# OnurBasci/Real_Time_Path_Tracing_With_SpatioTemporal_Filtering

Measured on AMD Instinct MI355X. Metric: Mray/s (closest-hit queries / whole-frame time: G-buffer + gradient + trace + a-trous), higher is better.
Workload: dtype f32

## Files before the change

### real_time_path_tracing_with_spatiotemporal_filtering_amd/csrc/api_context.hip

```cpp
#include "api_internal.hpp"

#include <atomic>

namespace rtpt_impl {

thread_local std::string g_err;

int fail(int code, const std::string& msg) {
  g_err = msg;
  return code;
}


size_t frame_blocks(const rtpt_ctx* c) {
  const size_t tiles = ((static_cast<size_t>(c->cfg.width) + 63) / 64) * ((static_cast<size_t>(c->cfg.row_end - c->cfg.row_begin) + 3) / 4);
  return std::max(tiles, static_cast<size_t>(c->n_cu > 0 ? c->n_cu : 256) * 8);
}
int ensure_stack_spill(rtpt_ctx* c, size_t blocks) {
  if (!c->scene.use_bvh) return RTPT_OK;
  const size_t depth = static_cast<size_t>(c->scene.tree.bvh_depth + 2 < 8 ? 8 : c->scene.tree.bvh_depth + 2);
  const size_t lds = std::min<size_t>(depth, static_cast<size_t>(c->bvh_stack_lds));
  if (depth <= lds || blocks <= c->stack_spill_blocks) return RTPT_OK;
  if (c->stack_spill.ptr) {
    hipError_t e = hipStreamSynchronize(c->stream);
// ... 111 lines not shown
  g.row_base = static_cast<int32_t>(c->cfg.row_begin);
  g.y0 = static_cast<int32_t>(y0);
  g.y1 = static_cast<int32_t>(y1);
  return g;
}

rt::SceneView scene_view(const rtpt_ctx* c) {
  rt::SceneView s;
  s.isect_id = static_cast<const float4*>(c->scene.isect_id.ptr);
  s.isect_leaf = static_cast<const float4*>(c->scene.isect_leaf.ptr);
  s.leaf_ids = static_cast<const uint32_t*>(c->scene.tree.leaf_order.ptr);
  s.shade = static_cast<const float4*>(c->scene.shade.ptr);
  s.nodes = static_cast<const rt::BvhNodeQ*>(c->scene.tree.nodes.ptr);
  s.bvh_grid = static_cast<const float*>(c->scene.bvh_grid_dev.ptr);
  s.n_tris = c->scene.n_tris;
  s.use_bvh = c->scene.use_bvh ? 1u : 0u;
  s.paired = (c->scene.tris_paired && !c->no_pairing) ? 1u : 0u;
  s.leaf_pairs = c->scene.tree.leaf_pairs ? 1u : 0u;
  s.stack_depth = static_cast<uint32_t>(c->scene.tree.bvh_depth + 2 < 8 ? 8 : c->scene.tree.bvh_depth + 2);
  s.stack_lds = std::min<uint32_t>(s.stack_depth, static_cast<uint32_t>(c->bvh_stack_lds));
  s.stack_spill = static_cast<uint32_t*>(c->stack_spill.ptr);
  s.materials = static_cast<const float4*>(c->scene.materials.ptr);
  s.n_base_tris = c->scene.n_base_tris ? c->scene.n_base_tris : 1u;
  return s;
}

rt::TexView tex_view(const rtpt_ctx* c) {
  rt::TexView t;
  t.records = static_cast<const float4*>(c->scene.textures.records.ptr);
  t.desc = static_cast<const rt::TexDesc*>(c->scene.textures.desc.ptr);
  t.texels = static_cast<const float4*>(c->scene.textures.texels.ptr);
  t.levels = static_cast<const uint32_t*>(c->scene.textures.levels.ptr);
  t.bounce_spread = c->tex_bounce_spread;
  return t;
}

bool screen_bounds(const rtpt_ctx* c, const double org[3], const double c0[3], const double c1[3], const double c2[3],
                   double p00, double p11, double jitter_px, rt::TriBounds* out) {
  if (c->scene.host_tris.empty() || c->scene.n_tris > static_cast<uint32_t>(rt::kCullMaxTris)) return false;
  const double W = c->cfg.width, H = c->cfg.height;
  for (uint32_t t = 0; t < c->scene.n_tris; t++) {
    double xmin = 1e30, xmax = -1e30, ymin = 1e30, ymax = -1e30;
    bool unbounded = false;
    for (int k = 0; k < 3; k++) {
      const float* P = c->scene.host_tris.data() + 9 * static_cast<size_t>(t) + 3 * k;
      const double r[3] = {P[0] - org[0], P[1] - org[1], P[2] - org[2]};
// ... 139 lines not shown
    HIP_TRY(hipSetDevice(dev));
  }
  rtpt_ctx* c = new (std::nothrow) rtpt_ctx();
  if (!c) return fail(RTPT_E_NOMEM, "host allocation failed");
  c->cfg = *cfg;
  c->device = dev;
  hipError_t e = hipStreamCreateWithFlags(&c->own_stream, hipStreamNonBlocking);
  if (e != hipSuccess) {
    delete c;
    return fail(RTPT_E_DEVICE, std::string("hipStreamCreate: ") + hipGetErrorString(e));
  }
  c->stream = c->own_stream;
  {
    hipDeviceProp_t prop;
    if (hipGetDeviceProperties(&prop, dev) == hipSuccess && prop.multiProcessorCount > 0) c->n_cu = prop.multiProcessorCount;
    e = rt::prepare_device_atrous();
    if (e == hipSuccess) e = rt::prepare_device_atrous_chain();
    if (e != hipSuccess) {
      rtpt_destroy(c);
      return fail(RTPT_E_DEVICE, std::string("hipFuncSetAttribute: ") + hipGetErrorString(e));
    }
  }
  if (const char* v = std::getenv("RTPT_NO_TRI_PAIRS")) c->no_pairing = std::atoi(v) != 0;
  if (const char* v = std::getenv("RTPT_HOST_REFIT")) c->host_refit = std::atoi(v) != 0;
  c->device_bvh = (cfg->flags & RTPT_FLAG_DEVICE_BVH_BUILD) != 0;
  c->device_bvh_sah = c->device_bvh && (cfg->flags & RTPT_FLAG_DEVICE_BVH_SAH) != 0;
  if (const char* v = std::getenv("RTPT_DEVICE_BVH")) {
    if (!std::strcmp(v, "sah"))
      c->device_bvh = c->device_bvh_sah = true;
    else
      c->device_bvh = c->device_bvh || std::atoi(v) != 0;
  }
  c->device_flatten = c->device_bvh && (cfg->flags & RTPT_FLAG_DEVICE_FLATTEN) != 0;
  if (const char* v = std::getenv("RTPT_LBVH_ORDER")) c->lbvh_by_height = !std::strcmp(v, "height");
  if (const char* v = std::getenv("RTPT_NO_TRACE_FUSION")) c->fuse_trace = std::atoi(v) == 0;
  if (const char* v = std::getenv("RTPT_NO_FRAME_REUSE")) c->frame_reuse = std::atoi(v) == 0;
  if (const char* v = std::getenv("RTPT_NO_REPROJ_REUSE")) c->reproj_reuse = std::atoi(v) == 0;
  if (const char* v = std::getenv("RTPT_TRACE_POOL")) c->trace_pool = std::atoi(v) != 0;
  if (const char* v = std::getenv("RTPT_TEX_BOUNCE_SPREAD")) {
    const float f = std::strtof(v, nullptr);
    if (f > 0.0f && f <= 64.0f) c->tex_bounce_spread = f;
  }
  if (const char* v = std::getenv("RTPT_PT_WINDOW")) c->trace_window = static_cast<uint32_t>(std::max(0, std::atoi(v)));
  if (const char* v = std::getenv("RTPT_CHAIN_G1")) c->filter_policy.chain_g_pin = std::atoi(v);
  if (const char* v = std::getenv("RTPT_CHAIN_GENERIC")) c->filter_policy.chain_generic = std::atoi(v);
  if (const char* v = std::getenv("RTPT_CHAIN_WG_PER_CU")) c->filter_policy.chain_wg_per_cu = std::atoi(v);
// ... 337 lines not shown
```

### real_time_path_tracing_with_spatiotemporal_filtering_amd/csrc/api_internal.hpp

```cpp
#pragma once
#include <hip/hip_runtime.h>

#include <algorithm>
#include <cmath>
#include <cstdio>
#include <cstdlib>
#include <cfloat>
#include <cstring>
#include <new>
#include <string>
#include <vector>

#include "../../include/rtpt.h"
#include "bvh.hpp"
#include "kernels.hpp"
#include "rtpt_math.hpp"


namespace rtpt_impl {


extern thread_local std::string g_err;
int fail(int code, const std::string& msg);

// ... 159 lines not shown
  int device = 0;
  int n_cu = 256;
  hipStream_t own_stream = nullptr;
  hipStream_t stream = nullptr;

  Buf color[4];
  Buf vis[2];
  int lut_cur = 0;
  Buf worldpos, gradient, depth, prev_pixel, hit_id, raycount;
  Buf moments[2], variance[2];
  Buf var_scale;
  Buf albedo, shaded;
  Buf path_queue[2], path_queue_count;
  Buf normals;
  FrameState frame;
  void* present_dst = nullptr;
  Rows present_rows;
  Buf ray_tab;
  float ray_tab_p00 = 0.f, ray_tab_p11 = 0.f;
  uint32_t ray_tab_w = 0, ray_tab_h = 0;

  Scene scene;
  bool no_pairing = false;
  bool host_refit = false;
  bool device_bvh = false;
  bool device_bvh_sah = false;
  bool lbvh_by_height = false;
  bool device_flatten = false;
  Buf bvh_build_scratch, bvh_build_header;
  hipEvent_t build_ev[2] = {nullptr, nullptr};
  Buf pair_word;
  struct XfStage {
    void* host = nullptr;
    size_t bytes = 0;
    hipEvent_t done = nullptr;
    bool pending = false;
  } xf_stage[2];
  int xf_stage_cur = 0;
  uint64_t upload_info[4] = {0, 0, 0, 0};

  bool tables_valid = false;
  uint32_t debug_mask = 0;
  hipEvent_t handoff_event = nullptr;

  rt::GbufferArgs pending_gb{};
  bool pending_gb_valid = false;
// ... 108 lines not shown
```

### real_time_path_tracing_with_spatiotemporal_filtering_amd/csrc/bvh.cpp

```cpp
#include "bvh.hpp"

#include <algorithm>
#include <cfloat>
#include <cmath>
#include <cstring>

namespace rt {
namespace {

struct Box {
  float mn[3], mx[3];
  void reset() {
    for (int a = 0; a < 3; a++) {
      mn[a] = FLT_MAX;
      mx[a] = -FLT_MAX;
    }
  }
  void grow(const float* p) {
    for (int a = 0; a < 3; a++) {
      mn[a] = std::min(mn[a], p[a]);
      mx[a] = std::max(mx[a], p[a]);
    }
  }
  void grow(const Box& b) {
// ... 3 lines not shown
    }
  }
  float half_area() const {
    float dx = mx[0] - mn[0], dy = mx[1] - mn[1], dz = mx[2] - mn[2];
    if (dx < 0.f) return 0.f;
    return dx * dy + dy * dz + dz * dx;
  }
};

struct Prim {
  Box box;
  float c[3];
  uint32_t id;
  uint32_t w;
};

struct Child {
  Box box;
  uint32_t idx;
  uint32_t cnt;
};

constexpr int kBins = kBvhBins;

struct Builder {
  std::vector<Prim> prims;
  Bvh* out;
  float pad;

  Child make_leaf(uint32_t lo, uint32_t hi) {
    Child c;
    c.box.reset();
    c.idx = static_cast<uint32_t>(out->leaf_order.size());
    c.cnt = 0;
    for (uint32_t i = lo; i < hi; i++) {
      c.box.grow(prims[i].box);
      for (uint32_t k = 0; k < prims[i].w; k++) out->leaf_order.push_back(prims[i].id + k);
      c.cnt += prims[i].w;
    }
    return c;
  }

  Child build(uint32_t lo, uint32_t hi, int depth) {
    out->max_depth = std::max(out->max_depth, depth);
    const uint32_t w = prims[lo].w;
    uint32_t n = (hi - lo) * w;
// ... 4 lines not shown
    cb.reset();
    bb.reset();
    for (uint32_t i = lo; i < hi; i++) {
      cb.grow(prims[i].c);
      bb.grow(prims[i].box);
    }
    uint32_t mid = lo;
    bool median = depth >= kBvhMaxDepth - 26;
    if (median && may_leaf) return make_leaf(lo, hi);
    if (!median) {
      float best_cost = FLT_MAX;
      int best_axis = -1, best_split = -1;
      for (int a = 0; a < 3; a++) {
        float ext = cb.mx[a] - cb.mn[a];
        if (!(ext > 0.f)) continue;
        Box bins[kBins];
        uint32_t cnt[kBins];
        for (int b = 0; b < kBins; b++) {
          bins[b].reset();
          cnt[b] = 0;
        }
        float scale = kBins / ext;
        for (uint32_t i = lo; i < hi; i++) {
          int b = std::min(kBins - 1, static_cast<int>((prims[i].c[a] - cb.mn[a]) * scale));
          bins[b].grow(prims[i].box);
          cnt[b] += w;
        }
        float right_area[kBins];
        uint32_t right_cnt[kBins];
        Box acc;
        acc.reset();
        uint32_t c = 0;
        for (int b = kBins - 1; b > 0; b--) {
          acc.grow(bins[b]);
          c += cnt[b];
          right_area[b] = acc.half_area();
          right_cnt[b] = c;
        }
        acc.reset();
        c = 0;
        for (int b = 0; b < kBins - 1; b++) {
          acc.grow(bins[b]);
          c += cnt[b];
          if (c == 0 || right_cnt[b + 1] == 0) continue;
          float cost = acc.half_area() * c + right_area[b + 1] * right_cnt[b + 1];
          if (cost < best_cost) {
            best_cost = cost;
            best_axis = a;
            best_split = b;
          }
        }
      }
      if (may_leaf && (best_axis < 0 || kNodeCost * bb.half_area() + best_cost >= static_cast<float>(n) * bb.half_area()))
        return make_leaf(lo, hi);
      if (best_axis >= 0) {
        float ext = cb.mx[best_axis] - cb.mn[best_axis];
        float scale = kBins / ext;
        float mn = cb.mn[best_axis];
        int axis = best_axis, split = best_split;
        auto it = std::partition(prims.begin() + lo, prims.begin() + hi, [&](const Prim& p) {
          int b = std::min(kBins - 1, static_cast<int>((p.c[axis] - mn) * scale));
          return b <= split;
        });
        mid = static_cast<uint32_t>(it - prims.begin());
      }
    }
    if (mid == lo || mid == hi) {
      int axis = 0;
      float best = -1.f;
      for (int a = 0; a < 3; a++) {
        float e = cb.mx[a] - cb.mn[a];
        if (e > best) {
          best = e;
          axis = a;
        }
      }
      mid = lo + (hi - lo) / 2;
      std::nth_element(prims.begin() + lo, prims.begin() + mid, prims.begin() + hi,
                       [axis](const Prim& x, const Prim& y) {
                         return x.c[axis] < y.c[axis] || (x.c[axis] == y.c[axis] && x.id < y.id);
                       });
    }

    uint32_t node_index = static_cast<uint32_t>(out->nodes.size());
// ... 192 lines not shown
```

### real_time_path_tracing_with_spatiotemporal_filtering_amd/csrc/closest_hit.hpp

```cpp
#pragma once

#include "device_common.hpp"

namespace rt {
namespace {

struct HitRec {
  float t;
  uint32_t id1;
  float u, v, ad;
};

#define RTPT_DIV_TH(a, b) ((a) / (b))
#define RTPT_DIV_SH(a, b) ((a) / (b))

#ifndef RTPT_TRACE_ITEMS
#define RTPT_TRACE_ITEMS 11
#endif

template <bool TIE_BREAK>
__device__ __forceinline__ void tri_test(f3 o, f3 d, float4 r0, float4 r1, float4 r2, uint32_t id1, HitRec& h) {
  f3 v0{r0.x, r0.y, r0.z}, e1{r0.w, r1.x, r1.y}, e2{r1.z, r1.w, r2.x}, n{r2.y, r2.z, r2.w};
  f3 tv = o - v0;
  const float dn = exact::dot(d, n);
// ... 90 lines not shown
  }
  {
    const float dn = exact::dot(d, nb);
    const uint32_t sm = f2u(dn) & 0x80000000u;
    const float tt = u2f(f2u(exact::dot(tv, nb)) ^ sm);
    const float u = u2f(f2u(exact::dot(e2b, c)) ^ sm);
    const float v = u2f(f2u(e2c) ^ sm);
    const float ad = __builtin_fabsf(dn);
    if ((u <= 0.0f) && (v >= 0.0f) && (v - u <= ad) && (tt < 0.0f)) {
      const float th = RTPT_DIV_TH(-tt, ad);
      bool better = th < h.t;
      better = better || (th == h.t && h.id1 != 0 && id1b < h.id1);
      if (better) {
        h.t = th;
        h.id1 = id1b;
        h.u = u;
        h.v = v;
        h.ad = ad;
      }
    }
  }
}

__device__ __forceinline__ void closest_hit_brute(const SceneView& sc, f3 o, f3 d, HitRec& h) {
  typedef float v4f __attribute__((ext_vector_type(4)));
  using cv4f = const __attribute__((address_space(4))) v4f;
  cv4f* rec = (cv4f*)sc.isect_id;
  const uint32_t n = sc.n_tris;
  constexpr int kBruteUnroll = 8;
  constexpr int kPairUnroll = 8;
  if (sc.paired) {
#pragma unroll kPairUnroll
    for (uint32_t i = 0; i < n; i += 2) {
      const v4f a0 = rec[3 * i], a1 = rec[3 * i + 1], a2 = rec[3 * i + 2], b1 = rec[3 * i + 4], b2 = rec[3 * i + 5];
      tri_pair_test(o, d, make_float4(a0.x, a0.y, a0.z, a0.w), make_float4(a1.x, a1.y, a1.z, a1.w), make_float4(a2.x, a2.y, a2.z, a2.w),
                    make_float4(b1.x, b1.y, b1.z, b1.w), make_float4(b2.x, b2.y, b2.z, b2.w), i + 1, h);
    }
    return;
  }
#pragma unroll kBruteUnroll
  for (uint32_t i = 0; i < n; i++) {
    const v4f a0 = rec[3 * i], a1 = rec[3 * i + 1], a2 = rec[3 * i + 2];
    tri_test<false>(o, d, make_float4(a0.x, a0.y, a0.z, a0.w), make_float4(a1.x, a1.y, a1.z, a1.w),
                    make_float4(a2.x, a2.y, a2.z, a2.w), i + 1, h);
  }
}

constexpr int kWaveW = 16, kWaveH = 4;
__device__ __forceinline__ uint32_t tile_pixel(int wave, uint32_t lane) {
  return ((lane >> 4) << 6) | (static_cast<uint32_t>(wave) << 4) | (lane & 15u);
}
__device__ __forceinline__ int wave_x0(int wave) { return kWaveW * wave; }
__device__ __forceinline__ unsigned long long span_candidates(const TriBounds* bounds, uint32_t n, int x0, int y0) {
// ... 150 lines not shown
      cur = cl;
    } else if (hr) {
      cur = cr;
    } else {
      cur = pop();
    }
  };
  while (cur != kSentinel) {
    while (true) {
      const bool walk = !(cur & kLeafBit);
      const unsigned long long mw = __ballot(walk);
      if (!mw) break;
      const int nw = __builtin_popcountll(mw), na = __builtin_popcountll(__ballot(true));
      if (na - nw >= kBvhLeafRatio * nw) break;
      if (walk) node_step();
    }
    if ((cur & kLeafBit) && cur != kSentinel) {
      test_leaf(cur);
      cur = pop();
    }
  }
}

template <int BVH>
__device__ __forceinline__ void closest_hit(const SceneView& sc, f3 o, f3 d, HitRec& h, uint32_t* stack, int tid,
                                            int nt = kThreads, int bucket = 0) {
  if (BVH)
    closest_hit_bvh<BVH == 2>(sc, o, d, h, stack, tid, nt, bucket);
  else
    closest_hit_brute(sc, o, d, h);
}

__device__ __forceinline__ f3 bary_point(f3 v0, f3 v1, f3 v2, float b0, float b1, float b2) {
  return f3{fmaf_(v2.x, b2, fmaf_(v1.x, b1, v0.x * b0)), fmaf_(v2.y, b2, fmaf_(v1.y, b1, v0.y * b0)),
            fmaf_(v2.z, b2, fmaf_(v1.z, b1, v0.z * b0))};
}

inline int scene_mode(const SceneView& sc) { return sc.use_bvh ? (sc.leaf_pairs ? 2 : 1) : 0; }

}
}
```

### real_time_path_tracing_with_spatiotemporal_filtering_amd/csrc/kernels.hip

```cpp
#include <cstdlib>

#include "atrous_comb.hpp"
#include "final_split.hpp"
#include "pathtrace_tile.hpp"
#include "select.hpp"

namespace rt {
namespace {

__global__ void k_scene_prepare(ScenePrepArgs a) {
  uint32_t i = blockIdx.x * blockDim.x + threadIdx.x;
  if (i >= a.n_tris) return;
  {
    const float* t = a.tris + 9 * static_cast<size_t>(i);
    f3 v0 = ld3(t), v1 = ld3(t + 3), v2 = ld3(t + 6);
    f3 e1 = v1 - v0, e2 = v2 - v0;
    f3 nn = exact::cross(e1, e2);
    a.isect_id[3 * i] = make_float4(v0.x, v0.y, v0.z, e1.x);
    a.isect_id[3 * i + 1] = make_float4(e1.y, e1.z, e2.x, e2.y);
    a.isect_id[3 * i + 2] = make_float4(e2.z, nn.x, nn.y, nn.z);
    f3 n = exact::normalize(nn);
    a.shade[3 * i] = make_float4(v0.x, v0.y, v0.z, n.x);
    a.shade[3 * i + 1] = make_float4(v1.x, v1.y, v1.z, n.y);
    a.shade[3 * i + 2] = make_float4(v2.x, v2.y, v2.z, n.z);
// ... 69 lines not shown
#if RTPT_TILE_TIMELINE
  TimelineScope tl_(0, blockIdx.y * gridDim.x + blockIdx.x);
#endif
  gbuffer_tile<BVH>(a, blockIdx.x, blockIdx.y, stack);
}

__global__ __launch_bounds__(kThreads) void k_gradient(GradientArgs a) {
  const int x = blockIdx.x * kBlockX + threadIdx.x;
  const int y = a.g.y0 + blockIdx.y * kBlockY + threadIdx.y;
  if (x >= a.g.W || y >= a.g.y1) return;
  const size_t i = static_cast<size_t>(y - a.g.row_base) * a.g.W + x;
  const uint32_t id = a.vis[i];
  const f3 wp = id ? xyz(a.worldpos[i]) : f3{0.f, 0.f, 0.f};
  store_gradient(a.grad, i, gradient_lambda(id, wp, a.lut, a.lut_prev, a.normal_tab, a.area_tab, ld3(a.cam), ld3(a.light), ld3(a.light_prev), ld3(a.color),
                                            ld3(a.color_prev)));
}

template <int BVH, bool COMPACT, bool DEMOD, int TEX, int SPEC>
__global__ __launch_bounds__(kPtThreads)
__attribute__((amdgpu_waves_per_eu(kPtBvhWaves, kPtBvhWaves)))
void k_pathtrace(PathtraceArgs a, TexView tex) {
  pathtrace_tile<BVH, COMPACT, false, DEMOD, TEX, SPEC>(a, tex);
}
template <bool COMPACT, bool DEMOD, int TEX, int SPEC>
__global__ __launch_bounds__(kPtThreads)
__attribute__((amdgpu_waves_per_eu(kPtWaves, kPtWaves)))
void k_pathtrace_small(PathtraceArgs a, TexView tex) {
  pathtrace_tile<0, COMPACT, false, DEMOD, TEX, SPEC>(a, tex);
}

template <int BVH, bool DEMOD, int TEX, int SPEC>
__global__ __launch_bounds__(kPtThreads)
__attribute__((amdgpu_waves_per_eu(kPtBvhWaves, kPtBvhWaves)))
void k_gbuffer_pathtrace(PathtraceArgs a, GbufferArgs g, TexView tex) {
  gbuffer_pathtrace_body<BVH, DEMOD, TEX, SPEC>(a, g, tex);
}
template <bool DEMOD, int TEX, int SPEC>
__global__ __launch_bounds__(kPtThreads)
__attribute__((amdgpu_waves_per_eu(kPtWaves, kPtWaves)))
void k_gbuffer_pathtrace_small(PathtraceArgs a, GbufferArgs g, TexView tex) {
  gbuffer_pathtrace_body<0, DEMOD, TEX, SPEC>(a, g, tex);
}

template <int CW>
__global__ __launch_bounds__(kPtThreads)
__attribute__((amdgpu_waves_per_eu(kPtWaves, kPtWaves)))
void k_pathtrace_final(PathtraceArgs a, TexView tex, AtrousArgs f, FinalSplit sp) {
  static_assert(kPtThreads == kShThreads && kPtRows == kShWaves, "the two bodies share the workgroup shape");
  const FinalRole r = final_role(sp, blockIdx.x);
  if (r.role == kFinalRoleTile) {
    pathtrace_tile<0, true, false, false, 0, 0, 1>(a, tex, r.index, sp.tiles_x, a.tiles_y);
  } else {
    extern __shared__ __attribute__((aligned(16))) unsigned char final_lds[];
    const bool front = r.role == kFinalRoleFront;
#if RTPT_TILE_TIMELINE
    FilterTimelineScope tl_(r.role, front ? r.index : sp.n_front + r.index);
#endif
    comb_items<CW, true, false, false, 1, false, false, true, true>(f, final_lds, r.index, front ? sp.n_front : sp.n_tail,
                                                                       front ? 0u : sp.front_items, front ? sp.front_items : sp.items);
  }
}

template <int BVH, int TEX, int SPEC>
__global__ __launch_bounds__(kPtThreads) void k_pathtrace_queue(PathtraceArgs a, TexView tex) {
  extern __shared__ __attribute__((aligned(16))) uint32_t stack[];
  PathState& st = *reinterpret_cast<PathState*>(stack);
  __shared__ uint32_t wave_cnt[kPtRows];
  __shared__ uint32_t q_base;
  __shared__ unsigned int block_rays;
  const int tid = threadIdx.y * kBlockX + threadIdx.x;
  const int wave = __builtin_amdgcn_readfirstlane(static_cast<int>(threadIdx.y));
  const uint32_t lane = threadIdx.x;
  if (tid == 0) block_rays = 0;
  const f3 light_c = ld3(a.light_c);
  const uint32_t region = blockIdx.x % kPathQueues;
  const uint32_t n_in = a.q_in_count[region];
  const size_t region_base = static_cast<size_t>(region) * a.queue_region;
  unsigned int rays = 0;
  for (uint32_t base = (blockIdx.x / kPathQueues) * kPtThreads; base < n_in; base += (gridDim.x / kPathQueues) * kPtThreads) {
    uint32_t pix = 0, rng = 0;
    f3 o{0.f, 0.f, 0.f}, d{0.f, 0.f, -1.f}, acc{1.f, 1.f, 1.f};
    bool alive = base + static_cast<uint32_t>(tid) < n_in;
    if (alive) {
      const float4* q = reinterpret_cast<const float4*>(a.q_in) + 3 * (region_base + base + tid);
      const float4 q0 = q[0], q1 = q[1], q2 = q[2];
      pix = __float_as_uint(q0.x);
      rng = __float_as_uint(q0.y);
      o = f3{q0.z, q0.w, q1.x};
      d = f3{q1.y, q1.z, q1.w};
      acc = f3{q2.x, q2.y, q2.z};
    }
    for (uint32_t seg = a.seg_begin; seg < a.seg_end; seg++) {
      if (alive) {
        HitRec h{a.tmax, 0u, 0.f, 0.f, 1.f};
        closest_hit<BVH>(a.scene, o, d, h, stack, tid, kPtThreads, 1 + static_cast<int>(seg));
        const int x = static_cast<int>(pix & 0xFFFFu), y = static_cast<int>(pix >> 16);
        if (y >= a.count_y0 && y < a.count_y1) rays++;
        if (shade_segment<TEX, BVH, (RTPT_TRACE_ITEMS & 8) && BVH == 0, SPEC>(a, h, seg, light_c, o, d, acc, rng, tex)) {
          alive = false;
          const size_t gi = static_cast<size_t>(y - a.g.row_base) * a.g.W + x;
          a.image[gi] = make_float4(acc.x, acc.y, acc.z, a.depth[gi]);
        }
      }
      if (seg + 1 >= a.seg_end) break;
      const unsigned long long live = __ballot(alive);
      if (lane == 0) wave_cnt[wave] = static_cast<uint32_t>(__builtin_popcountll(live));
      __syncthreads();
      uint32_t cbase = 0, total = 0;
#pragma unroll
      for (int w = 0; w < kPtRows; w++) {
        const uint32_t c = wave_cnt[w];
        if (w < wave) cbase += c;
        total += c;
      }
      if (total == 0) break;
      if (alive) {
        const uint32_t slot = cbase + __builtin_amdgcn_mbcnt_hi(static_cast<uint32_t>(live >> 32),
                                                              __builtin_amdgcn_mbcnt_lo(static_cast<uint32_t>(live), 0u));
// ... 102 lines not shown
  size_t dyn = stack_bytes > sizeof(PathState) ? stack_bytes : sizeof(PathState);
  if (fin) {
    if (gb || !pol || !fin->reproj_in || !pathtrace_takes_final(a, tex, specular)) std::abort();
    dyn = dyn > final_role_lds(*fin) ? dyn : final_role_lds(*fin);
  }
  PathtraceArgs b = a;
  b.tiles_y = tiles_y;
  b.multi_off = static_cast<uint32_t>(dyn / 4);
  const size_t dyn_queue = dyn;
  if (a.spp > 1) dyn += 4 * kPtThreads * 4;
  const uint32_t phase0 = a.first_window ? a.first_window : pt_first_window(a.scene.use_bvh != 0);
  const bool split = a.spp == 1 && a.compact && a.queue[0] && a.queue_count && a.max_segments > phase0 &&
                     (a.max_segments <= 2 * phase0 || a.queue[1]);
  b.seg_begin = 0;
  b.seg_end = split ? phase0 : a.max_segments;
  b.q_in = nullptr;
  b.q_in_count = nullptr;
  b.q_out = split ? a.queue[0] : nullptr;
  b.q_out_count = split ? a.queue_count : nullptr;
  if (split) (void)hipMemsetAsync(a.queue_count, 0, 2 * kPathQueues * sizeof(uint32_t), s);
  if (fin) {
    const FinalSplit sp = final_split(a, *fin, *pol, grid.x, tiles_y);
    const dim3 grid1(final_grid(sp));
    hipLaunchKernelGGL(k_pathtrace_final<kFinalRoleCw>, grid1, block, dyn, s, b, tex, *fin, sp);
  } else
#if RTPT_AB_VARIANTS
  if (pool) {
    if (gb)
      hipLaunchKernelGGL((k_pathtrace_pool<true>), grid, block, dyn, s, b, *gb);
    else
      hipLaunchKernelGGL((k_pathtrace_pool<false>), grid, block, dyn, s, b, GbufferArgs{});
  } else
#endif
  with_mode3(scene_mode(a.scene), [&](auto mode) {
    constexpr int M = decltype(mode)::value;
    with_bool(a.albedo != nullptr, [&](auto demod) {
      constexpr bool D = decltype(demod)::value;
      with_mode3(tex_mode(tex), [&](auto tmode) {
        constexpr int T = decltype(tmode)::value;
        with_mode3(spec_mode(specular), [&](auto spec) {
          constexpr int S = decltype(spec)::value;
          if (gb) {
            if constexpr (M != 0)
              hipLaunchKernelGGL((k_gbuffer_pathtrace<M, D, T, S>), grid, block, dyn, s, b, *gb, tex);
            else
              hipLaunchKernelGGL((k_gbuffer_pathtrace_small<D, T, S>), grid, block, dyn, s, b, *gb, tex);
            return;
          }
          with_bool(a.compact != 0, [&](auto compact) {
            constexpr bool C = decltype(compact)::value;
            if constexpr (M != 0)
              hipLaunchKernelGGL((k_pathtrace<M, C, D, T, S>), grid, block, dyn, s, b, tex);
            else
              hipLaunchKernelGGL((k_pathtrace_small<C, D, T, S>), grid, block, dyn, s, b, tex);
          });
        });
      });
    });
  });
  if (!split) return;
  const int n_cu = a.n_cu > 0 ? a.n_cu : 256;
  const dim3 qgrid(static_cast<uint32_t>(n_cu) * 8u);
  int cur = 0;
  for (uint32_t begin = phase0, len = phase0; begin < a.max_segments; begin += len, len *= 2, cur ^= 1) {
    const uint32_t end = begin + len < a.max_segments ? begin + len : a.max_segments;
    PathtraceArgs c = b;
    c.seg_begin = begin;
    c.seg_end = end;
    c.q_in = a.queue[cur];
    c.q_in_count = a.queue_count + cur * kPathQueues;
    const bool more = end < a.max_segments;
    c.q_out = more ? a.queue[cur ^ 1] : nullptr;
    c.q_out_count = more ? a.queue_count + (cur ^ 1) * kPathQueues : nullptr;
    if (more) (void)hipMemsetAsync(a.queue_count + (cur ^ 1) * kPathQueues, 0, kPathQueues * sizeof(uint32_t), s);
    with_mode3(scene_mode(a.scene), [&](auto mode) {
      with_mode3(tex_mode(tex), [&](auto tmode) {
        with_mode3(spec_mode(specular), [&](auto spec) {
          hipLaunchKernelGGL((k_pathtrace_queue<decltype(mode)::value, decltype(tmode)::value, decltype(spec)::value>), qgrid, block,
                             dyn_queue, s, c, tex);
        });
      });
    });
    if (end >= a.max_segments) break;
  }
}

}
```

### real_time_path_tracing_with_spatiotemporal_filtering_amd/csrc/kernels.hpp

```cpp
#pragma once

#include <hip/hip_runtime.h>
#include <stdint.h>

#include "bvh.hpp"
#include "texture.hpp"

namespace rt {

struct SceneView {
  const float4* isect_id;
  const float4* isect_leaf;
  const uint32_t* leaf_ids;
  const float4* shade;
  const BvhNodeQ* nodes;
  const float* bvh_grid;
  uint32_t n_tris;
  uint32_t use_bvh;
  uint32_t paired;
  uint32_t leaf_pairs;
  uint32_t stack_depth;
  uint32_t stack_lds;
  uint32_t* stack_spill;
  const float4* materials;
  uint32_t n_base_tris;
};

struct TexView {
  const float4* records;
  const TexDesc* desc;
  const float4* texels;
  const uint32_t* levels;
  float bounce_spread;
};

void launch_mip_downsample(float4* atlas, uint32_t src, uint32_t sw, uint32_t sh, uint32_t dst, hipStream_t s);

struct TriBounds {
  int16_t x0, y0, x1, y1;
};
constexpr int kCullMaxTris = 64;

struct FrameGeom {
  int32_t W, H;
  int32_t row_base;
  int32_t y0, y1;
};

struct GbufferArgs {
// ... 264 lines not shown
```

### real_time_path_tracing_with_spatiotemporal_filtering_amd/csrc/pathtrace_tile.hpp

```cpp
#pragma once

#include "gbuffer_tile.hpp"
#include "shade_segment.hpp"

namespace rt {
namespace {

constexpr int kPtRows = 4;
constexpr int kPtThreads = kBlockX * kPtRows;

__device__ __forceinline__ void enqueue_paths(const PathtraceArgs& a, uint32_t region, uint32_t* wave_cnt, uint32_t* bcast,
                                              bool alive, int wave, uint32_t lane, uint32_t pixg, uint32_t rng, f3 o, f3 d, f3 acc) {
  const unsigned long long m = __ballot(alive);
  if (lane == 0) wave_cnt[wave] = static_cast<uint32_t>(__builtin_popcountll(m));
  __syncthreads();
  uint32_t before = 0, total = 0;
#pragma unroll
  for (int w = 0; w < kPtRows; w++) {
    const uint32_t c = wave_cnt[w];
    if (w < wave) before += c;
    total += c;
  }
  if (wave == 0 && lane == 0) *bcast = total ? atomicAdd(a.q_out_count + region, total) : 0u;
  __syncthreads();
// ... 15 lines not shown
  float dx[kPtThreads], dy[kPtThreads], dz[kPtThreads];
  float ar[kPtThreads], ag[kPtThreads], ab[kPtThreads];
};

__device__ __forceinline__ void add_block_rays(const PathtraceArgs& a, unsigned int rays, unsigned int* block_rays, int tid, uint32_t slot) {
  for (int off = 32; off > 0; off >>= 1) rays += __shfl_down(rays, off, 64);
  if ((tid & 63) == 0 && rays) atomicAdd(block_rays, rays);
  __syncthreads();
  const unsigned int sum = *block_rays;
  if (tid == 0 && sum) atomicAdd(a.raycount + (slot & (kRayCounters - 1u)), static_cast<unsigned long long>(sum));
}

constexpr int kPtWaves = 8;
template <int ROLE>
__device__ __forceinline__ uint32_t tile_gx(uint32_t role_gx) {
  if constexpr (ROLE != 0) return role_gx;
  else return gridDim.x;
}
template <int ROLE>
__device__ __forceinline__ uint32_t tile_lin(uint32_t role_lin) {
  if constexpr (ROLE != 0) return role_lin;
  else return blockIdx.y * gridDim.x + blockIdx.x;
}
template <int BVH, bool COMPACT, bool GB, bool DEMOD, int TEX, int SPEC = 0, int ROLE = 0>
__device__ __forceinline__ void pathtrace_tile(const PathtraceArgs& a, const TexView& tex, const uint32_t role_lin = 0, const uint32_t role_gx = 0,
                                               const uint32_t role_gy = 0) {
  extern __shared__ __attribute__((aligned(16))) uint32_t stack[];
  PathState& st = *reinterpret_cast<PathState*>(stack);
  float* const sum_r = reinterpret_cast<float*>(stack + a.multi_off);
  float* const sum_g = sum_r + kPtThreads;
  float* const sum_b = sum_g + kPtThreads;
  uint32_t* const rng_pix = reinterpret_cast<uint32_t*>(sum_b + kPtThreads);
  __shared__ uint32_t wave_cnt[kPtRows];
  __shared__ uint32_t q_base;
  __shared__ unsigned int block_rays;
  const int tid = threadIdx.y * kBlockX + threadIdx.x;
  const int wave = __builtin_amdgcn_readfirstlane(static_cast<int>(threadIdx.y));
  const uint32_t lane = threadIdx.x;
  if (tid == 0) block_rays = 0;
  const uint32_t tiles_y_ = GB ? a.tiles_y : (ROLE ? role_gy : gridDim.y);
  const uint32_t lin_ = tile_lin<ROLE>(role_lin), col_ = lin_ / tiles_y_;
  uint32_t bx_ = (col_ & 1u) ? (tile_gx<ROLE>(role_gx) - 1u) / 2u + (col_ + 1u) / 2u : (tile_gx<ROLE>(role_gx) - 1u) / 2u - col_ / 2u, by_ = lin_ % tiles_y_;
#if RTPT_TILE_TIMELINE
  if (g_tile_order_n == tile_gx<ROLE>(role_gx) * (ROLE ? role_gy : gridDim.y)) {
    const uint32_t t_ = g_tile_order[lin_];
    bx_ = t_ % tile_gx<ROLE>(role_gx);
    by_ = t_ / tile_gx<ROLE>(role_gx);
// ... 25 lines not shown
    }
    const int px0 = tile_x0 + static_cast<int>(pix0 & 63u), py0 = tile_y0 + static_cast<int>(pix0 >> 6);
    bool alive = (px0 < a.g.W) && (py0 < a.g.y1);
    if (alive) {
      float u1 = glsl_max(1e-38f, exact::rng_next(rng));
      float u2 = exact::rng_next(rng);
      float rad = exact::sqrt_(-2.0f * exact::log_(u1));
      float sn, cs;
      exact::sincos2pi(u2, sn, cs);
      float cx = fmaf_(a.jitter, rad * cs, static_cast<float>(px0) + 0.5f);
      float cy = fmaf_(a.jitter, rad * sn, static_cast<float>(py0) + 0.5f);
      float ux = RTPT_DIV_SH(fmaf_(2.0f, cx, -fw), fh);
      float uy = -RTPT_DIV_SH(fmaf_(2.0f, cy, -fh), fh);
      d = exact::normalize(f3{a.slope * ux, a.slope * uy, -1.0f});
      o = ld3(a.cam);
      acc = f3{1.f, 1.f, 1.f};
    }
    for (uint32_t seg = 0; seg < a.seg_end; seg++) {
      if (alive) {
        HitRec h{a.tmax, 0u, 0.f, 0.f, 1.f};
        if (!BVH && a.cull && seg == 0)
          closest_hit_brute_set(a.scene, cand, o, d, h);
        else
          closest_hit<BVH>(a.scene, o, d, h, stack, tid, kPtThreads, 1 + static_cast<int>(seg));
        const int x = tile_x0 + static_cast<int>(pix & 63u), y = tile_y0 + static_cast<int>(pix >> 6);
        if (y >= a.count_y0 && y < a.count_y1) rays++;
        const size_t gi = static_cast<size_t>(y - a.g.row_base) * a.g.W + x;
        if (seg == 0 && smp == 0 && a.hit_id) a.hit_id[gi] = h.id1;
        constexpr bool kShortDiv = (RTPT_TRACE_ITEMS & 8) && BVH == 0 && COMPACT && !DEMOD;
        const bool done = shade_segment<TEX, BVH, kShortDiv, SPEC>(a, h, seg, light_c, o, d, acc, rng, tex, (DEMOD && seg == 0) ? a.albedo + gi : nullptr);
        if (done) {
          alive = false;
          if (a.spp == 1) {
            if (GB)
              store_rgb(a.image + gi, acc);
            else
              a.image[gi] = make_float4(acc.x, acc.y, acc.z, a.depth[gi]);
          } else {
            sum_r[pix] += acc.x;
            sum_g[pix] += acc.y;
            sum_b[pix] += acc.z;
            rng_pix[pix] = rng;
          }
        }
      }
      if (seg + 1 >= a.seg_end) break;
      if (!COMPACT) {
// ... 33 lines not shown
    }
    if (a.seg_end < a.max_segments) {
      const uint32_t pixg = (static_cast<uint32_t>(tile_y0 + static_cast<int>(pix >> 6)) << 16) |
                            static_cast<uint32_t>(tile_x0 + static_cast<int>(pix & 63u));
      const uint32_t blk = tile_lin<ROLE>(role_lin);
      enqueue_paths(a, blk % kPathQueues, wave_cnt, &q_base, alive, wave, lane, pixg, rng, o, d, acc);
    }
  }
  __syncthreads();
  if (a.spp > 1) {
    const int x = tile_x0 + static_cast<int>(lane), y = tile_y0 + wave;
    if (x < a.g.W && y < a.g.y1) {
      const float ns = static_cast<float>(a.spp);
      const size_t gi = static_cast<size_t>(y - a.g.row_base) * a.g.W + x;
      if (GB)
        store_rgb(a.image + gi, f3{sum_r[tid] / ns, sum_g[tid] / ns, sum_b[tid] / ns});
      else
        a.image[gi] = make_float4(sum_r[tid] / ns, sum_g[tid] / ns, sum_b[tid] / ns, a.depth[gi]);
    }
  }
  add_block_rays(a, rays, &block_rays, tid, tile_lin<ROLE>(role_lin));
}

template <int BVH, bool DEMOD, int TEX, int SPEC>
__device__ __forceinline__ void gbuffer_pathtrace_body(const PathtraceArgs& a, const GbufferArgs& g, const TexView& tex) {
  if (blockIdx.y < a.tiles_y) {
    pathtrace_tile<BVH, true, true, DEMOD, TEX, SPEC>(a, tex);
  } else {
    extern __shared__ __attribute__((aligned(16))) uint32_t stack[];
#if RTPT_TILE_TIMELINE
    TimelineScope tl_(0, (blockIdx.y - a.tiles_y) * gridDim.x + blockIdx.x);
#endif
    gbuffer_tile<BVH>(g, blockIdx.x, blockIdx.y - a.tiles_y, stack, a.image, a.g.y0, a.g.y1);
  }
}

constexpr int kPtBvhWaves = 8;

}
}
```

### real_time_path_tracing_with_spatiotemporal_filtering_amd/csrc/selftest_kernels.hip

```cpp
#include "closest_hit.hpp"
#include "dielectric.hpp"
#include "select.hpp"
#include "shade_segment.hpp"
#include "specular.hpp"
#include "texture.hpp"

namespace rt {
namespace {

__global__ void k_selftest_math(int op, const float* in, float* out, size_t n) {
  size_t i = static_cast<size_t>(blockIdx.x) * blockDim.x + threadIdx.x;
  if (i >= n) return;
  float x = in[i], r = 0.f, s, c;
  switch (op) {
    case 0: r = exact::log_(x); break;
    case 1: exact::sincos2pi(x, s, c); r = s; break;
    case 2: exact::sincos2pi(x, s, c); r = c; break;
    case 3: r = exact::sqrt_(x); break;
    case 4: r = exact::rcp_(x); break;
    case 5: r = fast::exp_(x); break;
    case 6: { uint32_t st = f2u(x); r = exact::rng_next(st); break; }
    case 7: r = exact::exp_(x); break;
    default: break;
  }
// ... 148 lines not shown

__global__ void k_selftest_bounce(const float* in, float* out, size_t n) {
  const size_t i = static_cast<size_t>(blockIdx.x) * blockDim.x + threadIdx.x;
  if (i >= n) return;
  const float* w = in + 9 * i;
  bool absorbed;
  const f3 dn = spec::bounce(ld3(w + 3), ld3(w), w[6], w[7], w[8], &absorbed);
  out[4 * i] = dn.x; out[4 * i + 1] = dn.y; out[4 * i + 2] = dn.z;
  out[4 * i + 3] = absorbed ? 1.0f : 0.0f;
}

__global__ void k_selftest_refract(const float* in, float* out, size_t n) {
  const size_t i = static_cast<size_t>(blockIdx.x) * blockDim.x + threadIdx.x;
  if (i >= n) return;
  const float* w = in + 9 * i;
  bool transmitted;
  float fresnel;
  const f3 dn = diel::refract(ld3(w + 3), ld3(w), w[6], w[8], &transmitted, &fresnel);
  out[5 * i] = dn.x; out[5 * i + 1] = dn.y; out[5 * i + 2] = dn.z;
  out[5 * i + 3] = transmitted ? 1.0f : 0.0f;
  out[5 * i + 4] = fresnel;
}

template <int BVH>
__global__ __launch_bounds__(kThreads) void k_selftest_trace(SceneView sc, const float* rays, size_t n, float tmax,
                                                             uint32_t* out_id, float* out_t) {
  extern __shared__ uint32_t stack[];
  size_t i = static_cast<size_t>(blockIdx.x) * kThreads + threadIdx.x;
  if (i >= n) return;
  f3 o = ld3(rays + 6 * i), d = ld3(rays + 6 * i + 3);
  HitRec h{tmax, 0u, 0.f, 0.f, 1.f};
  closest_hit<BVH>(sc, o, d, h, stack, threadIdx.x);
  out_id[i] = h.id1;
  if (out_t) out_t[i] = h.id1 ? h.t : 0.0f;
}

__global__ void k_selftest_texture(const TexDesc* desc, const float4* texels, const float* uv, size_t n, float4* out) {
  const size_t i = static_cast<size_t>(blockIdx.x) * blockDim.x + threadIdx.x;
  if (i >= n) return;
  out[i] = tex::sample(*desc, texels, uv[2 * i], uv[2 * i + 1]);
}

__global__ void k_selftest_texture_lod(const TexDesc* desc, const uint32_t* lv, const float4* texels, const float* uv, const float* lod,
                                       size_t n, float4* out) {
  const size_t i = static_cast<size_t>(blockIdx.x) * blockDim.x + threadIdx.x;
  if (i >= n) return;
  out[i] = tex::sample_lod(*desc, lv, texels, uv[2 * i], uv[2 * i + 1], lod[i]);
}

template <int BVH>
__global__ __launch_bounds__(kThreads) void k_selftest_footprint(SceneView sc, TexView tex, const float* rays, size_t n, float tmax,
                                                                 uint32_t primary, float slope, int frame_h, uint32_t* out_id,
                                                                 float* out_lod) {
  extern __shared__ uint32_t stack[];
  size_t i = static_cast<size_t>(blockIdx.x) * kThreads + threadIdx.x;
// ... 54 lines not shown
  hipLaunchKernelGGL(k_selftest_texture, dim3((n + 255) / 256), dim3(256), 0, s, desc, texels, uv, n, out);
}
void launch_selftest_texture_lod(const TexDesc* desc, const uint32_t* lv, const float4* texels, const float* uv, const float* lod, size_t n,
                                 float4* out, hipStream_t s) {
  if (!n) return;
  hipLaunchKernelGGL(k_selftest_texture_lod, dim3((n + 255) / 256), dim3(256), 0, s, desc, lv, texels, uv, lod, n, out);
}
void launch_selftest_footprint(const SceneView& scene, const TexView& tex, const float* rays, size_t n, float tmax, bool primary, float slope,
                               int frame_h, uint32_t* out_id, float* out_lod, hipStream_t s) {
  if (!n) return;
  dim3 grid((n + kThreads - 1) / kThreads), block(kThreads);
  with_mode3(scene_mode(scene), [&](auto mode) {
    constexpr int M = decltype(mode)::value;
    hipLaunchKernelGGL(k_selftest_footprint<M>, grid, block, M ? scene.stack_lds * kThreads * 4 : 0, s, scene, tex, rays, n, tmax,
                       primary ? 1u : 0u, slope, frame_h, out_id, out_lod);
  });
}
void launch_selftest_trace(const SceneView& scene, const float* rays, size_t n, float tmax, uint32_t* out_id,
                           float* out_t, hipStream_t s) {
  if (!n) return;
  dim3 grid((n + kThreads - 1) / kThreads), block(kThreads);
  with_mode3(scene_mode(scene), [&](auto mode) {
    constexpr int M = decltype(mode)::value;
    hipLaunchKernelGGL(k_selftest_trace<M>, grid, block, M ? scene.stack_lds * kThreads * 4 : 0, s, scene, rays, n, tmax, out_id, out_t);
  });
}

}
```

Measured before the change: 31960.

## Add two-pass brute-force closest-hit: branchless hit mask, then distance and winner UV

```diff
diff --git a/real_time_path_tracing_with_spatiotemporal_filtering_amd/csrc/api_context.hip b/real_time_path_tracing_with_spatiotemporal_filtering_amd/csrc/api_context.hip
--- a/real_time_path_tracing_with_spatiotemporal_filtering_amd/csrc/api_context.hip
+++ b/real_time_path_tracing_with_spatiotemporal_filtering_amd/csrc/api_context.hip
@@ -157,6 +157,7 @@
   s.stack_spill = static_cast<uint32_t*>(c->stack_spill.ptr);
   s.materials = static_cast<const float4*>(c->scene.materials.ptr);
   s.n_base_tris = c->scene.n_base_tris ? c->scene.n_base_tris : 1u;
+  s.brute_two_pass = c->no_brute_two_pass ? 0u : 1u;
   return s;
 }
 
@@ -342,6 +343,7 @@
     }
   }
   if (const char* v = std::getenv("RTPT_NO_TRI_PAIRS")) c->no_pairing = std::atoi(v) != 0;
+  if (const char* v = std::getenv("RTPT_NO_BRUTE_TWO_PASS")) c->no_brute_two_pass = std::atoi(v) != 0;
   if (const char* v = std::getenv("RTPT_HOST_REFIT")) c->host_refit = std::atoi(v) != 0;
   c->device_bvh = (cfg->flags & RTPT_FLAG_DEVICE_BVH_BUILD) != 0;
   c->device_bvh_sah = c->device_bvh && (cfg->flags & RTPT_FLAG_DEVICE_BVH_SAH) != 0;
diff --git a/real_time_path_tracing_with_spatiotemporal_filtering_amd/csrc/api_internal.hpp b/real_time_path_tracing_with_spatiotemporal_filtering_amd/csrc/api_internal.hpp
--- a/real_time_path_tracing_with_spatiotemporal_filtering_amd/csrc/api_internal.hpp
+++ b/real_time_path_tracing_with_spatiotemporal_filtering_amd/csrc/api_internal.hpp
@@ -205,6 +205,7 @@
 
   Scene scene;
   bool no_pairing = false;
+  bool no_brute_two_pass = false;
   bool host_refit = false;
   bool device_bvh = false;
   bool device_bvh_sah = false;
diff --git a/real_time_path_tracing_with_spatiotemporal_filtering_amd/csrc/bvh.cpp b/real_time_path_tracing_with_spatiotemporal_filtering_amd/csrc/bvh.cpp
--- a/real_time_path_tracing_with_spatiotemporal_filtering_amd/csrc/bvh.cpp
+++ b/real_time_path_tracing_with_spatiotemporal_filtering_amd/csrc/bvh.cpp
@@ -49,6 +49,7 @@
 };
 
 constexpr int kBins = kBvhBins;
+inline int sah_bin(float x) { return x >= 0.f ? (x < static_cast<float>(kBins) ? static_cast<int>(x) : kBins - 1) : 0; }
 
 struct Builder {
   std::vector<Prim> prims;
@@ -99,7 +100,7 @@
         }
         float scale = kBins / ext;
         for (uint32_t i = lo; i < hi; i++) {
-          int b = std::min(kBins - 1, static_cast<int>((prims[i].c[a] - cb.mn[a]) * scale));
+          int b = sah_bin((prims[i].c[a] - cb.mn[a]) * scale);
           bins[b].grow(prims[i].box);
           cnt[b] += w;
         }
@@ -136,7 +137,7 @@
         float mn = cb.mn[best_axis];
         int axis = best_axis, split = best_split;
         auto it = std::partition(prims.begin() + lo, prims.begin() + hi, [&](const Prim& p) {
-          int b = std::min(kBins - 1, static_cast<int>((p.c[axis] - mn) * scale));
+          int b = sah_bin((p.c[axis] - mn) * scale);
           return b <= split;
         });
         mid = static_cast<uint32_t>(it - prims.begin());
diff --git a/real_time_path_tracing_with_spatiotemporal_filtering_amd/csrc/closest_hit.hpp b/real_time_path_tracing_with_spatiotemporal_filtering_amd/csrc/closest_hit.hpp
--- a/real_time_path_tracing_with_spatiotemporal_filtering_amd/csrc/closest_hit.hpp
+++ b/real_time_path_tracing_with_spatiotemporal_filtering_amd/csrc/closest_hit.hpp
@@ -136,6 +136,97 @@
   }
 }
 
+__device__ __forceinline__ bool tri_ok(f3 o, f3 d, float4 r0, float4 r1, float4 r2) {
+  f3 v0{r0.x, r0.y, r0.z}, e1{r0.w, r1.x, r1.y}, e2{r1.z, r1.w, r2.x}, n{r2.y, r2.z, r2.w};
+  f3 tv = o - v0;
+  const float dn = exact::dot(d, n);
+  const uint32_t sm = f2u(dn) & 0x80000000u;
+  const float tt = u2f(f2u(exact::dot(tv, n)) ^ sm);
+  const f3 c = exact::cross(tv, d);
+  const float u = u2f(f2u(exact::dot(e2, c)) ^ sm);
+  const float v = u2f(f2u(exact::dot(e1, c)) ^ sm);
+  const float ad = __builtin_fabsf(dn);
+  return (u <= 0.0f) && (v >= 0.0f) && (v - u <= ad) && (tt < 0.0f);
+}
+__device__ __forceinline__ void tri_pair_ok(f3 o, f3 d, float4 r0, float4 r1, float4 r2, float4 q1, float4 q2, bool& ok_a, bool& ok_b) {
+  const f3 v0{r0.x, r0.y, r0.z}, e1{r0.w, r1.x, r1.y}, e2{r1.z, r1.w, r2.x}, n{r2.y, r2.z, r2.w};
+  const f3 e2b{q1.z, q1.w, q2.x}, nb{q2.y, q2.z, q2.w};
+  const f3 tv = o - v0;
+  const f3 c = exact::cross(tv, d);
+  const float e2c = exact::dot(e2, c);
+  {
+    const float dn = exact::dot(d, n);
+    const uint32_t sm = f2u(dn) & 0x80000000u;
+    const float tt = u2f(f2u(exact::dot(tv, n)) ^ sm);
+    const float u = u2f(f2u(e2c) ^ sm);
+    const float v = u2f(f2u(exact::dot(e1, c)) ^ sm);
+    const float ad = __builtin_fabsf(dn);
+    ok_a = (u <= 0.0f) && (v >= 0.0f) && (v - u <= ad) && (tt < 0.0f);
+  }
+  {
+    const float dn = exact::dot(d, nb);
+    const uint32_t sm = f2u(dn) & 0x80000000u;
+    const float tt = u2f(f2u(exact::dot(tv, nb)) ^ sm);
+    const float u = u2f(f2u(exact::dot(e2b, c)) ^ sm);
+    const float v = u2f(f2u(e2c) ^ sm);
+    const float ad = __builtin_fabsf(dn);
+    ok_b = (u <= 0.0f) && (v >= 0.0f) && (v - u <= ad) && (tt < 0.0f);
+  }
+}
+
+#ifndef RTPT_BRUTE_UV_EACH
+#define RTPT_BRUTE_UV_EACH 0
+#endif
+
+__device__ __forceinline__ void brute_candidates(const SceneView& sc, uint32_t base, uint32_t mask, f3 o, f3 d, HitRec& h, uint32_t& win) {
+#if !RTPT_BRUTE_UV_EACH
+  float best = h.t;
+#endif
+  while (mask) {
+    const uint32_t i = base + static_cast<uint32_t>(__builtin_ctz(mask));
+    mask &= mask - 1u;
+    const float4* r = reinterpret_cast<const float4*>(reinterpret_cast<const unsigned char*>(sc.isect_id) + __umul24(i, 48u));
+#if RTPT_BRUTE_UV_EACH
+    tri_test<false>(o, d, r[0], r[1], r[2], i + 1, h);
+#else
+    const float4 r0 = r[0], r2 = r[2];
+    const f3 v0{r0.x, r0.y, r0.z}, n{r2.y, r2.z, r2.w};
+    const f3 tv = o - v0;
+    const float dn = exact::dot(d, n);
+    const uint32_t sm = f2u(dn) & 0x80000000u;
+    const float tt = u2f(f2u(exact::dot(tv, n)) ^ sm);
+    const float ad = __builtin_fabsf(dn);
+    const float th = RTPT_DIV_TH(-tt, ad);
+    if (th < best) {
+      best = th;
+      win = i + 1;
+    }
+#endif
+  }
+#if !RTPT_BRUTE_UV_EACH
+  h.t = best;
+#endif
+}
+
+__device__ __forceinline__ void brute_winner(const SceneView& sc, uint32_t win, f3 o, f3 d, HitRec& h) {
+#if !RTPT_BRUTE_UV_EACH
+  if (win) {
+    const float4* r = reinterpret_cast<const float4*>(reinterpret_cast<const unsigned char*>(sc.isect_id) + __umul24(win - 1u, 48u));
+    const float4 r0 = r[0], r1 = r[1], r2 = r[2];
+    const f3 v0{r0.x, r0.y, r0.z}, e1{r0.w, r1.x, r1.y}, e2{r1.z, r1.w, r2.x}, n{r2.y, r2.z, r2.w};
+    const f3 tv = o - v0;
+    const float dn = exact::dot(d, n);
+    const uint32_t sm = f2u(dn) & 0x80000000u;
+    const f3 c = exact::cross(tv, d);
+    h.id1 = win;
+    h.u = u2f(f2u(exact::dot(e2, c)) ^ sm);
+    h.v = u2f(f2u(exact::dot(e1, c)) ^ sm);
+    h.ad = __builtin_fabsf(dn);
+  }
+#endif
+}
+
+template <bool TWO_PASS = false>
 __device__ __forceinline__ void closest_hit_brute(const SceneView& sc, f3 o, f3 d, HitRec& h) {
   typedef float v4f __attribute__((ext_vector_type(4)));
   using cv4f = const __attribute__((address_space(4))) v4f;
@@ -143,6 +234,33 @@
   const uint32_t n = sc.n_tris;
   constexpr int kBruteUnroll = 8;
   constexpr int kPairUnroll = 8;
+  if constexpr (TWO_PASS) {
+    uint32_t win = 0;
+    for (uint32_t base = 0; base < n; base += 32) {
+      const uint32_t end = n - base < 32u ? n : base + 32u;
+      uint32_t mask = 0;
+      if (sc.paired) {
+#pragma unroll kPairUnroll
+        for (uint32_t i = base; i < end; i += 2) {
+          const v4f a0 = rec[3 * i], a1 = rec[3 * i + 1], a2 = rec[3 * i + 2], b1 = rec[3 * i + 4], b2 = rec[3 * i + 5];
+          bool ok_a, ok_b;
+          tri_pair_ok(o, d, make_float4(a0.x, a0.y, a0.z, a0.w), make_float4(a1.x, a1.y, a1.z, a1.w), make_float4(a2.x, a2.y, a2.z, a2.w),
+                      make_float4(b1.x, b1.y, b1.z, b1.w), make_float4(b2.x, b2.y, b2.z, b2.w), ok_a, ok_b);
+          mask |= ((ok_a ? 1u : 0u) | (ok_b ? 2u : 0u)) << (i - base);
+        }
+      } else {
+#pragma unroll kBruteUnroll
+        for (uint32_t i = base; i < end; i++) {
+          const v4f a0 = rec[3 * i], a1 = rec[3 * i + 1], a2 = rec[3 * i + 2];
+          const bool ok = tri_ok(o, d, make_float4(a0.x, a0.y, a0.z, a0.w), make_float4(a1.x, a1.y, a1.z, a1.w), make_float4(a2.x, a2.y, a2.z, a2.w));
+          mask |= (ok ? 1u : 0u) << (i - base);
+        }
+      }
+      brute_candidates(sc, base, mask, o, d, h, win);
+    }
+    brute_winner(sc, win, o, d, h);
+    return;
+  }
   if (sc.paired) {
 #pragma unroll kPairUnroll
     for (uint32_t i = 0; i < n; i += 2) {
@@ -339,13 +457,13 @@
   }
 }
 
-template <int BVH>
+template <int BVH, bool TWO_PASS = false>
 __device__ __forceinline__ void closest_hit(const SceneView& sc, f3 o, f3 d, HitRec& h, uint32_t* stack, int tid,
                                             int nt = kThreads, int bucket = 0) {
   if (BVH)
     closest_hit_bvh<BVH == 2>(sc, o, d, h, stack, tid, nt, bucket);
   else
-    closest_hit_brute(sc, o, d, h);
+    closest_hit_brute<TWO_PASS>(sc, o, d, h);
 }
 
 __device__ __forceinline__ f3 bary_point(f3 v0, f3 v1, f3 v2, float b0, float b1, float b2) {
@@ -354,6 +472,7 @@
 }
 
 inline int scene_mode(const SceneView& sc) { return sc.use_bvh ? (sc.leaf_pairs ? 2 : 1) : 0; }
-
-}
-}
+inline bool brute_two_pass(const SceneView& sc) { return !sc.use_bvh && sc.brute_two_pass; }
+
+}
+}
diff --git a/real_time_path_tracing_with_spatiotemporal_filtering_amd/csrc/kernels.hip b/real_time_path_tracing_with_spatiotemporal_filtering_amd/csrc/kernels.hip
--- a/real_time_path_tracing_with_spatiotemporal_filtering_amd/csrc/kernels.hip
+++ b/real_time_path_tracing_with_spatiotemporal_filtering_amd/csrc/kernels.hip
@@ -115,11 +115,11 @@
 void k_pathtrace(PathtraceArgs a, TexView tex) {
   pathtrace_tile<BVH, COMPACT, false, DEMOD, TEX, SPEC>(a, tex);
 }
-template <bool COMPACT, bool DEMOD, int TEX, int SPEC>
+template <bool COMPACT, bool DEMOD, int TEX, int SPEC, bool TP>
 __global__ __launch_bounds__(kPtThreads)
 __attribute__((amdgpu_waves_per_eu(kPtWaves, kPtWaves)))
 void k_pathtrace_small(PathtraceArgs a, TexView tex) {
-  pathtrace_tile<0, COMPACT, false, DEMOD, TEX, SPEC>(a, tex);
+  pathtrace_tile<0, COMPACT, false, DEMOD, TEX, SPEC, 0, TP>(a, tex);
 }
 
 template <int BVH, bool DEMOD, int TEX, int SPEC>
@@ -128,21 +128,21 @@
 void k_gbuffer_pathtrace(PathtraceArgs a, GbufferArgs g, TexView tex) {
   gbuffer_pathtrace_body<BVH, DEMOD, TEX, SPEC>(a, g, tex);
 }
-template <bool DEMOD, int TEX, int SPEC>
+template <bool DEMOD, int TEX, int SPEC, bool TP>
 __global__ __launch_bounds__(kPtThreads)
 __attribute__((amdgpu_waves_per_eu(kPtWaves, kPtWaves)))
 void k_gbuffer_pathtrace_small(PathtraceArgs a, GbufferArgs g, TexView tex) {
-  gbuffer_pathtrace_body<0, DEMOD, TEX, SPEC>(a, g, tex);
-}
-
-template <int CW>
+  gbuffer_pathtrace_body<0, DEMOD, TEX, SPEC, TP>(a, g, tex);
+}
+
+template <int CW, bool TP>
 __global__ __launch_bounds__(kPtThreads)
 __attribute__((amdgpu_waves_per_eu(kPtWaves, kPtWaves)))
 void k_pathtrace_final(PathtraceArgs a, TexView tex, AtrousArgs f, FinalSplit sp) {
   static_assert(kPtThreads == kShThreads && kPtRows == kShWaves, "the two bodies share the workgroup shape");
   const FinalRole r = final_role(sp, blockIdx.x);
   if (r.role == kFinalRoleTile) {
-    pathtrace_tile<0, true, false, false, 0, 0, 1>(a, tex, r.index, sp.tiles_x, a.tiles_y);
+    pathtrace_tile<0, true, false, false, 0, 0, 1, TP>(a, tex, r.index, sp.tiles_x, a.tiles_y);
   } else {
     extern __shared__ __attribute__((aligned(16))) unsigned char final_lds[];
     const bool front = r.role == kFinalRoleFront;
@@ -154,7 +154,7 @@
   }
 }
 
-template <int BVH, int TEX, int SPEC>
+template <int BVH, int TEX, int SPEC, bool TP>
 __global__ __launch_bounds__(kPtThreads) void k_pathtrace_queue(PathtraceArgs a, TexView tex) {
   extern __shared__ __attribute__((aligned(16))) uint32_t stack[];
   PathState& st = *reinterpret_cast<PathState*>(stack);
@@ -186,7 +186,7 @@
     for (uint32_t seg = a.seg_begin; seg < a.seg_end; seg++) {
       if (alive) {
         HitRec h{a.tmax, 0u, 0.f, 0.f, 1.f};
-        closest_hit<BVH>(a.scene, o, d, h, stack, tid, kPtThreads, 1 + static_cast<int>(seg));
+        closest_hit<BVH, TP>(a.scene, o, d, h, stack, tid, kPtThreads, 1 + static_cast<int>(seg));
         const int x = static_cast<int>(pix & 0xFFFFu), y = static_cast<int>(pix >> 16);
         if (y >= a.count_y0 && y < a.count_y1) rays++;
         if (shade_segment<TEX, BVH, (RTPT_TRACE_ITEMS & 8) && BVH == 0, SPEC>(a, h, seg, light_c, o, d, acc, rng, tex)) {
@@ -335,7 +335,9 @@
   if (fin) {
     const FinalSplit sp = final_split(a, *fin, *pol, grid.x, tiles_y);
     const dim3 grid1(final_grid(sp));
-    hipLaunchKernelGGL(k_pathtrace_final<kFinalRoleCw>, grid1, block, dyn, s, b, tex, *fin, sp);
+    with_bool(brute_two_pass(a.scene), [&](auto tp) {
+      hipLaunchKernelGGL((k_pathtrace_final<kFinalRoleCw, decltype(tp)::value>), grid1, block, dyn, s, b, tex, *fin, sp);
+    });
   } else
 #if RTPT_AB_VARIANTS
   if (pool) {
@@ -357,7 +359,10 @@
             if constexpr (M != 0)
               hipLaunchKernelGGL((k_gbuffer_pathtrace<M, D, T, S>), grid, block, dyn, s, b, *gb, tex);
             else
-              hipLaunchKernelGGL((k_gbuffer_pathtrace_small<D, T, S>), grid, block, dyn, s, b, *gb, tex);
+              with_bool(T == 0 && brute_two_pass(a.scene), [&](auto tp) {
+                if constexpr (T == 0 || !decltype(tp)::value)
+                  hipLaunchKernelGGL((k_gbuffer_pathtrace_small<D, T, S, decltype(tp)::value>), grid, block, dyn, s, b, *gb, tex);
+              });
             return;
           }
           with_bool(a.compact != 0, [&](auto compact) {
@@ -365,7 +370,10 @@
             if constexpr (M != 0)
               hipLaunchKernelGGL((k_pathtrace<M, C, D, T, S>), grid, block, dyn, s, b, tex);
             else
-              hipLaunchKernelGGL((k_pathtrace_small<C, D, T, S>), grid, block, dyn, s, b, tex);
+              with_bool(C && T == 0 && brute_two_pass(a.scene), [&](auto tp) {
+                if constexpr ((C && T == 0) || !decltype(tp)::value)
+                  hipLaunchKernelGGL((k_pathtrace_small<C, D, T, S, decltype(tp)::value>), grid, block, dyn, s, b, tex);
+              });
           });
         });
       });
@@ -389,8 +397,12 @@
     with_mode3(scene_mode(a.scene), [&](auto mode) {
       with_mode3(tex_mode(tex), [&](auto tmode) {
         with_mode3(spec_mode(specular), [&](auto spec) {
-          hipLaunchKernelGGL((k_pathtrace_queue<decltype(mode)::value, decltype(tmode)::value, decltype(spec)::value>), qgrid, block,
-                             dyn_queue, s, c, tex);
+          constexpr int M = decltype(mode)::value;
+          with_bool(M == 0 && brute_two_pass(a.scene), [&](auto tp) {
+            if constexpr (M == 0 || !decltype(tp)::value)
+              hipLaunchKernelGGL((k_pathtrace_queue<M, decltype(tmode)::value, decltype(spec)::value, decltype(tp)::value>), qgrid, block,
+                                 dyn_queue, s, c, tex);
+          });
         });
       });
     });
diff --git a/real_time_path_tracing_with_spatiotemporal_filtering_amd/csrc/kernels.hpp b/real_time_path_tracing_with_spatiotemporal_filtering_amd/csrc/kernels.hpp
--- a/real_time_path_tracing_with_spatiotemporal_filtering_amd/csrc/kernels.hpp
+++ b/real_time_path_tracing_with_spatiotemporal_filtering_amd/csrc/kernels.hpp
@@ -24,7 +24,9 @@
   uint32_t* stack_spill;
   const float4* materials;
   uint32_t n_base_tris;
-};
+  uint32_t brute_two_pass;
+};
+static_assert(sizeof(SceneView) == 96, "brute_two_pass fills the tail padding");
 
 struct TexView {
   const float4* records;
diff --git a/real_time_path_tracing_with_spatiotemporal_filtering_amd/csrc/pathtrace_tile.hpp b/real_time_path_tracing_with_spatiotemporal_filtering_amd/csrc/pathtrace_tile.hpp
--- a/real_time_path_tracing_with_spatiotemporal_filtering_amd/csrc/pathtrace_tile.hpp
+++ b/real_time_path_tracing_with_spatiotemporal_filtering_amd/csrc/pathtrace_tile.hpp
@@ -61,7 +61,7 @@
   if constexpr (ROLE != 0) return role_lin;
   else return blockIdx.y * gridDim.x + blockIdx.x;
 }
-template <int BVH, bool COMPACT, bool GB, bool DEMOD, int TEX, int SPEC = 0, int ROLE = 0>
+template <int BVH, bool COMPACT, bool GB, bool DEMOD, int TEX, int SPEC = 0, int ROLE = 0, bool TP = false>
 __device__ __forceinline__ void pathtrace_tile(const PathtraceArgs& a, const TexView& tex, const uint32_t role_lin = 0, const uint32_t role_gx = 0,
                                                const uint32_t role_gy = 0) {
   extern __shared__ __attribute__((aligned(16))) uint32_t stack[];
@@ -133,7 +133,7 @@
         if (!BVH && a.cull && seg == 0)
           closest_hit_brute_set(a.scene, cand, o, d, h);
         else
-          closest_hit<BVH>(a.scene, o, d, h, stack, tid, kPtThreads, 1 + static_cast<int>(seg));
+          closest_hit<BVH, TP>(a.scene, o, d, h, stack, tid, kPtThreads, 1 + static_cast<int>(seg));
         const int x = tile_x0 + static_cast<int>(pix & 63u), y = tile_y0 + static_cast<int>(pix >> 6);
         if (y >= a.count_y0 && y < a.count_y1) rays++;
         const size_t gi = static_cast<size_t>(y - a.g.row_base) * a.g.W + x;
@@ -213,10 +213,10 @@
   add_block_rays(a, rays, &block_rays, tid, tile_lin<ROLE>(role_lin));
 }
 
-template <int BVH, bool DEMOD, int TEX, int SPEC>
+template <int BVH, bool DEMOD, int TEX, int SPEC, bool TP = false>
 __device__ __forceinline__ void gbuffer_pathtrace_body(const PathtraceArgs& a, const GbufferArgs& g, const TexView& tex) {
   if (blockIdx.y < a.tiles_y) {
-    pathtrace_tile<BVH, true, true, DEMOD, TEX, SPEC>(a, tex);
+    pathtrace_tile<BVH, true, true, DEMOD, TEX, SPEC, 0, TP>(a, tex);
   } else {
     extern __shared__ __attribute__((aligned(16))) uint32_t stack[];
 #if RTPT_TILE_TIMELINE
diff --git a/real_time_path_tracing_with_spatiotemporal_filtering_amd/csrc/selftest_kernels.hip b/real_time_path_tracing_with_spatiotemporal_filtering_amd/csrc/selftest_kernels.hip
--- a/real_time_path_tracing_with_spatiotemporal_filtering_amd/csrc/selftest_kernels.hip
+++ b/real_time_path_tracing_with_spatiotemporal_filtering_amd/csrc/selftest_kernels.hip
@@ -194,7 +194,7 @@
   out[5 * i + 4] = fresnel;
 }
 
-template <int BVH>
+template <int BVH, bool TP>
 __global__ __launch_bounds__(kThreads) void k_selftest_trace(SceneView sc, const float* rays, size_t n, float tmax,
                                                              uint32_t* out_id, float* out_t) {
   extern __shared__ uint32_t stack[];
@@ -202,7 +202,7 @@
   if (i >= n) return;
   f3 o = ld3(rays + 6 * i), d = ld3(rays + 6 * i + 3);
   HitRec h{tmax, 0u, 0.f, 0.f, 1.f};
-  closest_hit<BVH>(sc, o, d, h, stack, threadIdx.x);
+  closest_hit<BVH, TP>(sc, o, d, h, stack, threadIdx.x);
   out_id[i] = h.id1;
   if (out_t) out_t[i] = h.id1 ? h.t : 0.0f;
 }
@@ -303,7 +303,11 @@
   dim3 grid((n + kThreads - 1) / kThreads), block(kThreads);
   with_mode3(scene_mode(scene), [&](auto mode) {
     constexpr int M = decltype(mode)::value;
-    hipLaunchKernelGGL(k_selftest_trace<M>, grid, block, M ? scene.stack_lds * kThreads * 4 : 0, s, scene, rays, n, tmax, out_id, out_t);
+    with_bool(M == 0 && brute_two_pass(scene), [&](auto tp) {
+      if constexpr (M == 0 || !decltype(tp)::value)
+        hipLaunchKernelGGL((k_selftest_trace<M, decltype(tp)::value>), grid, block, M ? scene.stack_lds * kThreads * 4 : 0, s, scene, rays, n, tmax,
+                           out_id, out_t);
+    });
   });
 }
 
```

New measurement: 32200 (median of 6 runs). About the same (+0.8%).
